# tanushreebanerjee/generative-detection

Hardware: AMD Instinct MI355X
Metric: VAE train images/s (fwd+bwd+opt) at 256x256 z=16x16x16 (higher is better)
Workload: dtype f32; 1 GPU; autoencoder_kl_16x16x16.yaml, 256x256 synthetic crops, B=32/GPU, rec+KL only (discriminator off, optimizer 0), fp32, VAE phase; global_batch=32, parallelism=dp1

## Files before the change

generative-detection_amd/csrc/bf16_common.h:

```cpp
#pragma once
#include "common.h"

typedef unsigned short bf16_t;
typedef __bf16 bf16x8 __attribute__((ext_vector_type(8)));
typedef short s16x4 __attribute__((ext_vector_type(4)));
typedef unsigned int u32x2 __attribute__((ext_vector_type(2)));

__device__ __forceinline__ float bf16_to_f32(bf16_t v) { return __uint_as_float((unsigned)v << 16); }
__device__ __forceinline__ bf16_t f32_to_bf16(float f) {
  unsigned u = __float_as_uint(f);
  if ((u & 0x7FFFFFFFu) > 0x7F800000u) return (bf16_t)((u >> 16) | 0x40);
  u += 0x7FFFu + ((u >> 16) & 1u);
  return (bf16_t)(u >> 16);
}
__device__ __forceinline__ unsigned pack_bf16x2(float lo, float hi) {
#if defined(__HIP_DEVICE_COMPILE__)
  unsigned r;
  asm("v_cvt_pk_bf16_f32 %0, %1, %2" : "=v"(r) : "v"(lo), "v"(hi));
  return r;
#else
  (void)lo; (void)hi; return 0;
#endif
}
__device__ __forceinline__ float bf16_lo(unsigned w) { return __uint_as_float(w << 16); }
__device__ __forceinline__ float bf16_hi(unsigned w) { return __uint_as_float(w & 0xFFFF0000u); }

__device__ __forceinline__ f32x16 mfma_bf16(bf16x8 a, bf16x8 b, f32x16 c) {
#if defined(__HIP_DEVICE_COMPILE__)
  return __builtin_amdgcn_mfma_f32_32x32x16_bf16(a, b, c, 0, 0, 0);
#else
  (void)a; (void)b; return c;
#endif
}
__device__ __forceinline__ bf16x8 frag_from_u32x4(u32x4 v) { return __builtin_bit_cast(bf16x8, v); }

__device__ __forceinline__ s16x4 lds_read_tr16(const bf16_t* lds_addr) {
#if defined(__HIP_DEVICE_COMPILE__)
  return __builtin_amdgcn_ds_read_tr16_b64_v4i16((s16x4 __attribute__((address_space(3)))*)lds_addr);
#else
  (void)lds_addr; return s16x4{0, 0, 0, 0};
#endif
}
__device__ __forceinline__ bf16x8 frag_from_tr(s16x4 lo, s16x4 hi) {
  typedef short s16x8 __attribute__((ext_vector_type(8)));
  s16x8 v = {lo[0], lo[1], lo[2], lo[3], hi[0], hi[1], hi[2], hi[3]};
  return __builtin_bit_cast(bf16x8, v);
}

typedef __attribute__((address_space(3))) char lds_char_t;
__device__ __forceinline__ unsigned lds_addr_of(const void* generic) { return (unsigned)(uintptr_t)(lds_char_t*)generic; }
__device__ __forceinline__ u32x4 lds_ld128(unsigned a) { return *(const __attribute__((address_space(3))) u32x4*)(uintptr_t)a; }
__device__ __forceinline__ f32x4 lds_ld128f(unsigned a) { return *(const __attribute__((address_space(3))) f32x4*)(uintptr_t)a; }
__device__ __forceinline__ void lds_st128(unsigned a, u32x4 v) { *(__attribute__((address_space(3))) u32x4*)(uintptr_t)a = v; }
__device__ __forceinline__ void lds_st128f(unsigned a, f32x4 v) { *(__attribute__((address_space(3))) f32x4*)(uintptr_t)a = v; }
__device__ __forceinline__ s16x4 lds_ld_tr(unsigned a) {
#if defined(__HIP_DEVICE_COMPILE__)
  return __builtin_amdgcn_ds_read_tr16_b64_v4i16((s16x4 __attribute__((address_space(3)))*)(uintptr_t)a);
#else
  (void)a; return s16x4{0, 0, 0, 0};
#endif
}

typedef int i32x4_t __attribute__((ext_vector_type(4)));
__device__ __forceinline__ i32x4_t rsrc_words(const void* base, unsigned bytes) {
  const uint64_t a = (uint64_t)base;
  i32x4_t r;
  r.x = (int)(unsigned)a; r.y = (int)((unsigned)(a >> 32) & 0xFFFFu); r.z = (int)bytes; r.w = 0x00020000;
  return r;
}
__device__ __forceinline__ void lds_dma16(i32x4_t rsrc, unsigned lds_dst, unsigned voff) {
#if defined(__HIP_DEVICE_COMPILE__)
  unsigned keep;
  asm volatile("s_mov_b32 %0, m0\n\ts_mov_b32 m0, %2\n\ts_nop 0\n\tbuffer_load_dwordx4 %1, %3, 0 offen lds\n\ts_mov_b32 m0, %0"
               : "=&s"(keep) : "v"(voff), "s"(lds_dst), "s"(rsrc) : "memory");
#else
  (void)rsrc; (void)lds_dst; (void)voff;
#endif
}
__device__ __forceinline__ void lds_dma16_s(i32x4_t rsrc, unsigned lds_dst, unsigned voff, unsigned soff) {
// ... 18 lines not shown
```

generative-detection_amd/csrc/conv3x3_wgrad_wino_f32.hip:

```cpp
#include "common.h"

namespace {

constexpr int CT = 16;
constexpr int RS = 128;
constexpr int OPF = 4 * CT * RS;
constexpr unsigned OOB = 0xFFFFFFF0u;

struct WgwParams {
  const float* x; const float* dy; float* slabs; float* bias_part;
  int N, H, W, Cin, Cout, TY, TX;
  int total_tiles, total_chunks, chunks_per_split, nsplit;
};

__device__ __forceinline__ float4 f4(u32x4 v) {
  return make_float4(__uint_as_float(v.x), __uint_as_float(v.y), __uint_as_float(v.z), __uint_as_float(v.w));
}
template <int A, int B>
__device__ __forceinline__ float4 f4lin(float4 x, float4 y) {
  static_assert(A >= -1 && A <= 1 && B >= -1 && B <= 1 && (A != 0 || B != 0), "coefficients are -1, 0 or 1");
  if constexpr (B == 0) return A > 0 ? x : make_float4(-x.x, -x.y, -x.z, -x.w);
  else if constexpr (A == 0) return B > 0 ? y : make_float4(-y.x, -y.y, -y.z, -y.w);
  else if constexpr (A > 0 && B > 0) return make_float4(x.x + y.x, x.y + y.y, x.z + y.z, x.w + y.w);
  else if constexpr (A > 0) return make_float4(x.x - y.x, x.y - y.y, x.z - y.z, x.w - y.w);
  else if constexpr (B > 0) return make_float4(y.x - x.x, y.y - x.y, y.z - x.z, y.w - x.w);
  else return make_float4(-x.x - y.x, -x.y - y.y, -x.z - y.z, -x.w - y.w);
}
__device__ __forceinline__ float4 f4add(float4 a, float4 b) { return make_float4(a.x + b.x, a.y + b.y, a.z + b.z, a.w + b.w); }
__device__ __forceinline__ float4 f4sub(float4 a, float4 b) { return make_float4(a.x - b.x, a.y - b.y, a.z - b.z, a.w - b.w); }

template <bool WIDE, int R>
__device__ __forceinline__ void wgw_body(const WgwParams& p, float* dsm, const int split) {
  const int tid = threadIdx.x, lane = tid & 63;
  const int wave = __builtin_amdgcn_readfirstlane(tid >> 6);
  const int cig = wave & 3, coh = wave >> 2;
  const int li = lane & 31, h = lane >> 5;
  constexpr int r = R;
  const int cib = blockIdx.y, cob = blockIdx.z;
  constexpr int ra = r == 0 ? 0 : 1, rb = r == 3 ? 3 : 2;
  constexpr int sa = r == 2 ? -1 : 1, sb = (r == 0 || r == 3) ? -1 : 1;
  constexpr int ya = r == 3 ? 0 : 1, yb = r == 0 ? 0 : (r == 1 ? 1 : -1);

  const __amdgpu_buffer_rsrc_t xrsrc = __builtin_amdgcn_make_buffer_rsrc(
      const_cast<float*>(p.x), 0, (unsigned)((int64_t)p.N * p.H * p.W * p.Cin * 4), 0x00020000);
  const __amdgpu_buffer_rsrc_t yrsrc = __builtin_amdgcn_make_buffer_rsrc(
      const_cast<float*>(p.dy), 0, (unsigned)((int64_t)p.N * p.H * p.W * p.Cout * 4), 0x00020000);

  const int chunk0 = split * p.chunks_per_split;
  const int nch = min(p.chunks_per_split, p.total_chunks - chunk0);
  const int end_tile = min(p.total_tiles, (chunk0 + nch) * CT);

  const int st = tid >> 5, sq = tid & 31;
  int tl = chunk0 * CT + st, tn, tty, ttx;
// ... 128 lines not shown
    __builtin_amdgcn_sched_barrier(0);
    mm(1); fetch_y();
    __builtin_amdgcn_sched_barrier(0);
    ldf(va, mb, 5, 1);
    __builtin_amdgcn_sched_barrier(0);
    mm(0);
    __builtin_amdgcn_sched_barrier(0);
    ldf(va, mb, 6, 0);
    __builtin_amdgcn_sched_barrier(0);
    mm(1);
    __builtin_amdgcn_sched_barrier(0);
    ldf(va, mb, 7, 1);
    __builtin_amdgcn_sched_barrier(0);
    mm(0);
    mm(1);
    __syncthreads();
  }

#pragma unroll
  for (int c = 0; c < 4; ++c) {
    float* sl = p.slabs + ((int64_t)(split * 16 + 4 * r + c) * p.Cin + cib * 128 + cig * 32) * p.Cout + cob * 128 + coh * 64 + li;
#pragma unroll
    for (int nt = 0; nt < 2; ++nt)
#pragma unroll
      for (int q = 0; q < 16; ++q) sl[(int64_t)acc_row(q, lane) * p.Cout + nt * 32] = acc[c][nt][q];
  }
  if (r == 1 && cib == 0 && p.bias_part) {
    *reinterpret_cast<float4*>(dsm + st * 128 + 4 * sq) = bias_acc;
    __syncthreads();
    if (tid < 128) {
      float s = 0.f;
#pragma unroll
      for (int t = 0; t < CT; ++t) s += dsm[t * 128 + tid];
      p.bias_part[(int64_t)split * p.Cout + cob * 128 + tid] = s;
    }
  }
}

template <bool WIDE>
__global__ __launch_bounds__(512, 2) void conv3x3_wgrad_wino_kernel(WgwParams p) {
  extern __shared__ __attribute__((aligned(16))) float dsm[];
  const int bx = blockIdx.x;
  const bool xcd_map = (p.nsplit & 7) == 0;
  const int r = xcd_map ? (bx >> 3) & 3 : bx & 3;
  const int split = xcd_map ? (bx & 7) + 8 * (bx >> 5) : bx >> 2;
  switch (r) {
    case 0: wgw_body<WIDE, 0>(p, dsm, split); break;
    case 1: wgw_body<WIDE, 1>(p, dsm, split); break;
    case 2: wgw_body<WIDE, 2>(p, dsm, split); break;
    default: wgw_body<WIDE, 3>(p, dsm, split); break;
  }
}

__global__ __launch_bounds__(256) void conv3x3_wgrad_wino_reduce_kernel(const float* __restrict__ slabs, const float* __restrict__ bias_part,
                                                                        int nsplit, int Cin, int Cout, float* __restrict__ dw, float* __restrict__ db) {
  __shared__ float part[4][16][64];
  const int pl = threadIdx.x & 63, k = threadIdx.x >> 6;
  const int idx = blockIdx.x * 64 + pl;
  const bool live = idx < Cin * Cout;
  const int co = live ? idx % Cout : 0, ci = live ? idx / Cout : 0;
  float u[16];
#pragma unroll
  for (int xi = 0; xi < 16; ++xi) u[xi] = 0.f;
  if (live)
    for (int s = k; s < nsplit; s += 4)
#pragma unroll
      for (int xi = 0; xi < 16; ++xi) u[xi] += slabs[((int64_t)(s * 16 + xi) * Cin + ci) * Cout + co];
#pragma unroll
  for (int xi = 0; xi < 16; ++xi) part[k][xi][pl] = u[xi];
  __syncthreads();
  if (k != 0) return;
  if (live) {
#pragma unroll
    for (int xi = 0; xi < 16; ++xi) u[xi] = (part[0][xi][pl] + part[1][xi][pl]) + (part[2][xi][pl] + part[3][xi][pl]);
    float t[3][4];
#pragma unroll
    for (int j = 0; j < 4; ++j) {
      const float hs = 0.5f * (u[4 + j] + u[8 + j]), hd = 0.5f * (u[4 + j] - u[8 + j]);
      t[0][j] = u[j] + hs; t[1][j] = hd; t[2][j] = hs + u[12 + j];
    }
    float* o = dw + ((int64_t)co * Cin + ci) * 9;
#pragma unroll
    for (int a = 0; a < 3; ++a) {
      const float hs = 0.5f * (t[a][1] + t[a][2]), hd = 0.5f * (t[a][1] - t[a][2]);
      o[a * 3 + 0] = t[a][0] + hs; o[a * 3 + 1] = hd; o[a * 3 + 2] = hs + t[a][3];
    }
  }
  if (db && idx < Cout) {
    float sb = 0.f;
    for (int q = 0; q < nsplit; ++q) sb += bias_part[(int64_t)q * Cout + idx];
    db[idx] = sb;
  }
}

void plan(int N, int H, int W, int Cin, int Cout, WgwParams& p) {
  p.N = N; p.H = H; p.W = W; p.Cin = Cin; p.Cout = Cout; p.TY = H / 2; p.TX = W / 2;
  p.total_tiles = N * p.TY * p.TX;
  p.total_chunks = ceil_div(p.total_tiles, CT);
  const int base = 4 * (Cin / 128) * (Cout / 128);
  int ns = std::max(1, std::min(256 / base, p.total_chunks));
  p.chunks_per_split = ceil_div(p.total_chunks, ns);
  p.nsplit = ceil_div(p.total_chunks, p.chunks_per_split);
}

}

extern "C" {

int odvae_conv3x3_wgrad_wino_supported(int N, int H, int W, int Cin, int Cout) {
  if (N <= 0 || H <= 0 || W <= 0 || H % 2 || W % 2 || Cin <= 0 || Cout <= 0 || Cin % 128 || Cout % 128) return 0;
  const int64_t px = (int64_t)N * H * W;
  if (px * Cin * 4 >= (int64_t)OOB || px * Cout * 4 >= (int64_t)OOB || px / 4 >= (1ll << 30)) return 0;
  return 1;
}

size_t odvae_conv3x3_wgrad_wino_workspace_bytes(int N, int H, int W, int Cin, int Cout) {
  if (!odvae_conv3x3_wgrad_wino_supported(N, H, W, Cin, Cout)) return 0;
  WgwParams p; plan(N, H, W, Cin, Cout, p);
  return ((size_t)p.nsplit * 16 * Cin * Cout + (size_t)p.nsplit * Cout) * sizeof(float);
}

int odvae_conv3x3_wgrad_wino_f32(const float* x, const float* dy, int N, int H, int W, int Cin, int Cout,
                                 float* dw, float* dbias, void* workspace, size_t workspace_bytes, void* stream) {
  ODVAE_CHECK_ARG(x && dy && dw, "conv3x3_wgrad_wino: null operand");
  ODVAE_CHECK_ARG(odvae_conv3x3_wgrad_wino_supported(N, H, W, Cin, Cout),
                  "conv3x3_wgrad_wino: unsupported shape N=%d H=%d W=%d Cin=%d Cout=%d (even H, W; channels in multiples of 128; "
                  "tensors below 4 GiB)", N, H, W, Cin, Cout);
  ODVAE_CHECK_ARG(((uintptr_t)x & 15) == 0 && ((uintptr_t)dy & 15) == 0, "conv3x3_wgrad_wino: x/dy must be 16-byte aligned");
  WgwParams p; plan(N, H, W, Cin, Cout, p);
  const size_t need = odvae_conv3x3_wgrad_wino_workspace_bytes(N, H, W, Cin, Cout);
  if (!workspace || workspace_bytes < need) {
    odvae_set_error("conv3x3_wgrad_wino: workspace %zu < %zu bytes", workspace_bytes, need);
    return ODVAE_ERR_WORKSPACE;
  }
  p.x = x; p.dy = dy;
  p.slabs = static_cast<float*>(workspace);
  p.bias_part = dbias ? p.slabs + (size_t)p.nsplit * 16 * Cin * Cout : nullptr;
  const size_t smem = (size_t)4 * OPF * sizeof(float);
  auto kern = p.TX >= CT ? conv3x3_wgrad_wino_kernel<true> : conv3x3_wgrad_wino_kernel<false>;
  const hipError_t e = hipFuncSetAttribute(reinterpret_cast<const void*>(kern), hipFuncAttributeMaxDynamicSharedMemorySize, (int)smem);
  if (e != hipSuccess) {
    odvae_set_error("conv3x3_wgrad_wino: hipFuncSetAttribute failed: %s", hipGetErrorString(e));
    return ODVAE_ERR_HIP;
  }
  hipStream_t s = static_cast<hipStream_t>(stream);
  hipLaunchKernelGGL(kern, dim3(4 * p.nsplit, Cin / 128, Cout / 128), dim3(512), smem, s, p);
  ODVAE_LAUNCH_CHECK("conv3x3_wgrad_wino");
  const int pairs = Cin * Cout;
  hipLaunchKernelGGL(conv3x3_wgrad_wino_reduce_kernel, dim3(ceil_div(pairs, 64)), dim3(256), 0, s,
                     p.slabs, p.bias_part, p.nsplit, Cin, Cout, dw, dbias);
  ODVAE_LAUNCH_CHECK("conv3x3_wgrad_wino_reduce");
  return ODVAE_OK;
}

}
```

generative-detection_amd/csrc/gemm_f32_split.hip:

```cpp
#include "gemm_f32_tile.h"

namespace {

using namespace gemm_tile;

constexpr unsigned PLANE_B = BM * BK * 2;
constexpr unsigned OPER_B = 3 * PLANE_B;
constexpr unsigned OOB = 0x7FFFFFF0u;
constexpr int HI = 0, MID = 1, LO = 2;

__device__ __forceinline__ unsigned tile_byte(int row, int slot) {
  const int f = ((row >> 2) & 1) | ((((row >> 1) ^ (row >> 3)) & 1) << 1);
  return (unsigned)(row * 64 + ((slot ^ f) << 4));
}

__device__ __forceinline__ unsigned cvt_pk_bf16(float first, float second) {
  typedef float f32x2 __attribute__((ext_vector_type(2)));
  typedef __bf16 bf16x2 __attribute__((ext_vector_type(2)));
  return __builtin_bit_cast(unsigned, __builtin_convertvector(f32x2{first, second}, bf16x2));
}

__device__ __forceinline__ void split8(const float (&x)[8], u32x4 (&pl)[3]) {
#pragma unroll
  for (int j = 0; j < 4; ++j) {
    const float x0 = x[2 * j], x1 = x[2 * j + 1];
    const unsigned h = cvt_pk_bf16(x0, x1);
    const float r0 = x0 - bf16_lo(h), r1 = x1 - bf16_hi(h);
    const unsigned m = cvt_pk_bf16(r0, r1);
    const float s0 = r0 - bf16_lo(m), s1 = r1 - bf16_hi(m);
    pl[HI][j] = h; pl[MID][j] = m; pl[LO][j] = cvt_pk_bf16(s0, s1);
  }
}
__device__ __forceinline__ void store_unit(unsigned lds_oper, int row, int slot, const float (&x)[8]) {
  u32x4 pl[3];
  split8(x, pl);
  const unsigned a = lds_oper + tile_byte(row, slot);
#pragma unroll
  for (int q = 0; q < 3; ++q) lds_st128(a + q * PLANE_B, pl[q]);
}

template <bool KC>
struct SplitLoader {
  __amdgpu_buffer_rsrc_t rsrc;
  unsigned voff[2];
  unsigned ld_bytes;
  int kvalid;
  float x[2][8];

  __device__ __forceinline__ void init(const float* G, int ld, int row0, int nrows, int K) {
    const int tid = threadIdx.x;
    kvalid = K;
    ld_bytes = (unsigned)ld * 4u;
    if (KC) {
      const int rows = min(BM, nrows - row0);
      const int64_t bytes = ((int64_t)(rows - 1) * ld + K) * 4;
      rsrc = __builtin_amdgcn_make_buffer_rsrc(const_cast<float*>(G) + (int64_t)row0 * ld, 0, (int)(bytes < 0x7FFFFFF0ll ? bytes : 0x7FFFFFF0ll), 0x00020000);
#pragma unroll
      for (int i = 0; i < 2; ++i) {
        const int u = tid + 256 * i;
        voff[i] = (u >> 2) < rows ? (unsigned)(((u >> 2) * ld + 8 * (u & 3)) * 4) : OOB;
      }
    } else {
      const int64_t bytes = ((int64_t)(K - 1) * ld + (nrows - row0)) * 4;
      rsrc = __builtin_amdgcn_make_buffer_rsrc(const_cast<float*>(G) + row0, 0, (int)(bytes < 0x7FFFFFF0ll ? bytes : 0x7FFFFFF0ll), 0x00020000);
      const int row = tid & 127;
      voff[0] = row0 + row < nrows ? (unsigned)((tid >> 7) * 8 * ld + row) * 4u : OOB;
      voff[1] = 0;
    }
  }
  template <bool TAIL>
  __device__ __forceinline__ void load(int k0) {
    const int tid = threadIdx.x;
    const bool tail = TAIL && k0 + BK > kvalid;
    if (KC) {
      const unsigned soff = (unsigned)__builtin_amdgcn_readfirstlane(k0) * 4u;
#pragma unroll
      for (int i = 0; i < 2; ++i)
#pragma unroll
        for (int q = 0; q < 2; ++q) {
          unsigned vo = voff[i] + 16u * q;
          if (tail && k0 + 8 * ((tid + 256 * i) & 3) + 4 * q >= kvalid) vo = OOB;
          const u32x4 v = __builtin_amdgcn_raw_buffer_load_b128(rsrc, vo, soff, 0);
          x[i][4 * q] = __uint_as_float(v.x); x[i][4 * q + 1] = __uint_as_float(v.y);
          x[i][4 * q + 2] = __uint_as_float(v.z); x[i][4 * q + 3] = __uint_as_float(v.w);
        }
// ... 173 lines not shown
```

generative-detection_amd/lib.py:

```python
import ctypes
import os
import re

import torch

_HERE = os.path.dirname(os.path.abspath(__file__))
LIB_PATH = os.path.join(_HERE, "libodvae_hip.so")
HEADER_PATH = os.path.join(os.path.dirname(_HERE), "include", "odvae_hip.h")

_c = ctypes
_P, _I, _L, _F, _Z = _c.c_void_p, _c.c_int, _c.c_int64, _c.c_float, _c.c_size_t

ABI_VERSION = 4

PROTOTYPES = {
    "odvae_last_error": (_c.c_char_p, []),
    "odvae_abi_version": (_I, []),
    "odvae_target_arch": (_c.c_char_p, []),
    "odvae_gemm_f32_workspace_bytes": (_Z, [_I, _I, _I, _I]),
    "odvae_gemm_select_staging": (_I, [_I]),
    "odvae_gemm_f32": (_I, [_I, _I, _I, _I, _I, _F, _P, _I, _L, _P, _I, _L, _P, _I, _L, _P, _P, _I, _P, _Z, _P]),
    "odvae_gemm_softmax_bwd_f32": (_I, [_I, _I, _I, _F, _P, _I, _L, _P, _I, _L, _P, _P, _L, _P, _I, _L, _I, _P]),
    "odvae_rowdot_f32": (_I, [_P, _P, _L, _I, _P, _P]),
    "odvae_attn_row_bound_f32": (_I, [_P, _I, _I, _I, _P, _P, _P, _P]),
    "odvae_gemm_exp_bound_f32": (_I, [_I, _I, _I, _F, _P, _I, _L, _P, _I, _L, _P, _L, _P, _I, _L, _I, _P]),
    "odvae_gemm_rownorm_f32": (_I, [_I, _I, _I, _P, _I, _L, _P, _I, _L, _P, _I, _L, _P, _L, _P, _I, _P]),
    "odvae_gemm_pred_f32": (_I, [_I, _I, _I, _I, _I, _F, _P, _I, _L, _P, _I, _L, _P, _I, _L, _I, _P, _P]),
    "odvae_softmax_rows_pred_f32": (_I, [_P, _P, _L, _I, _F, _P, _P, _P]),
    "odvae_rowdot_scale_f32": (_I, [_P, _P, _P, _L, _I, _P, _P, _P]),
    "odvae_gemm_softmax_bwd_scaled_f32": (_I, [_I, _I, _I, _F, _P, _I, _L, _P, _I, _L, _P, _P, _P, _L, _P, _I, _L, _I, _P]),
    "odvae_conv3x3_pack_reduce_pad": (_I, [_I]),
    "odvae_conv3x3_pack_out_pad": (_I, [_I]),
    "odvae_conv3x3_pack_floats": (_Z, [_I, _I]),
    "odvae_conv3x3_pack_f32": (_I, [_P, _I, _I, _P, _P, _P]),
    "odvae_conv3x3_up_pack_floats": (_Z, [_I, _I]),
    "odvae_conv3x3_pack_up_f32": (_I, [_P, _I, _I, _P, _P, _P]),
    "odvae_conv3x3_wino_reduce_pad": (_I, [_I]),
    "odvae_conv3x3_wino_out_pad": (_I, [_I]),
    "odvae_conv3x3_wino_pack_floats": (_Z, [_I, _I]),
    "odvae_conv3x3_pack_wino_f32": (_I, [_P, _I, _I, _P, _P, _P]),
    "odvae_conv3x3_wino_f32": (_I, [_P, _I, _I, _I, _I, _P, _I, _P, _P, _P, _I, _P]),
    "odvae_conv3x3_wino4_reduce_pad": (_I, [_I]),
    "odvae_conv3x3_wino4_out_pad": (_I, [_I]),
    "odvae_conv3x3_wino4_pack_floats": (_Z, [_I, _I]),
    "odvae_conv3x3_wino4_supported": (_I, [_I, _I, _I, _I]),
    "odvae_conv3x3_pack_wino4_f32": (_I, [_P, _I, _I, _P, _P, _P]),
    "odvae_conv3x3_pack_wino_batch": (_I, [_P, _I, _P]),
    "odvae_conv3x3_pack_wino4_batch": (_I, [_P, _I, _P]),
    "odvae_conv3x3_wino4_f32": (_I, [_P, _I, _I, _I, _I, _P, _I, _P, _P, _P, _I, _P]),
    "odvae_conv3x3_wino4_stats_chunks": (_I, [_I, _I]),
    "odvae_conv3x3_wino4_stats_f32": (_I, [_P, _I, _I, _I, _I, _P, _I, _P, _P, _P, _P, _I, _P]),
    "odvae_conv3x3_wino4_up_f32": (_I, [_P, _I, _I, _I, _I, _P, _I, _P, _P, _P, _P, _I, _P]),
    "odvae_conv3x3_wino4_pool_f32": (_I, [_P, _I, _I, _I, _I, _P, _I, _P, _P]),
    "odvae_conv3x3_wino4_gnbwd_f32": (_I, [_P, _I, _I, _I, _I, _P, _I, _P, _P, _P, _P, _P, _P, _I, _P, _P]),
    "odvae_conv3x3_f32": (_I, [_I, _P, _I, _I, _I, _I, _P, _I, _P, _P, _P, _I, _I, _I, _P]),
    "odvae_conv3x3_wgrad_workspace_bytes": (_Z, [_I, _I, _I, _I, _I, _I]),
    "odvae_conv3x3_wgrad_f32": (_I, [_I, _P, _P, _I, _I, _I, _I, _I, _I, _I, _P, _P, _P, _Z, _P]),
    "odvae_conv3x3_wgrad_wino_supported": (_I, [_I, _I, _I, _I, _I]),
    "odvae_conv3x3_wgrad_wino_workspace_bytes": (_Z, [_I, _I, _I, _I, _I]),
    "odvae_conv3x3_wgrad_wino_f32": (_I, [_P, _P, _I, _I, _I, _I, _I, _P, _P, _P, _Z, _P]),
    "odvae_groupnorm_workspace_bytes": (_Z, [_I, _I, _I, _I]),
    "odvae_groupnorm_fwd_f32": (_I, [_P, _I, _I, _I, _I, _P, _P, _F, _I, _P, _P, _P, _P, _Z, _P]),
    "odvae_groupnorm_fwd_partials_f32": (_I, [_P, _I, _I, _I, _I, _P, _P, _F, _I, _P, _P, _P, _P, _I, _P]),
    "odvae_groupnorm_apply_f32": (_I, [_P, _I, _I, _I, _I, _P, _P, _P, _P, _I, _P, _P]),
    "odvae_groupnorm_apply_bf16": (_I, [_P, _I, _I, _I, _I, _P, _P, _P, _P, _I, _P, _P]),
    "odvae_groupnorm_bwd_f32": (_I, [_P, _P, _I, _I, _I, _I, _P, _P, _P, _P, _I, _P, _P, _P, _P, _P, _Z, _P]),
    "odvae_groupnorm_bwd_partials_f32": (_I, [_P, _P, _I, _I, _I, _I, _P, _P, _P, _P, _I, _P, _P, _P, _P, _P, _I, _P, _Z, _P]),
    "odvae_groupnorm_select_backward": (_I, [_I]),
    "odvae_groupnorm_fused_timeouts": (_I, []),
    "odvae_device_health": (_I, [_P, _P, _I, _I]),
    "odvae_attn_softmax_fallbacks": (_I, [_I]),
    "odvae_softmax_rows_f32": (_I, [_P, _P, _L, _I, _F, _P]),
    "odvae_softmax_rows_bwd_f32": (_I, [_P, _P, _P, _L, _I, _F, _P]),
    "odvae_upsample2x_bwd_f32": (_I, [_P, _P, _I, _I, _I, _I, _P]),
    "odvae_rescale_minmax_f32": (_I, [_P, _P, _I, _I, _I, _P, _P, _Z, _P]),
    "odvae_gaussian_sample_f32": (_I, [_P, _P, _P, _I, _I, _I, _P]),
    "odvae_gaussian_kl_f32": (_I, [_P, _P, _I, _I, _I, _P]),
    "odvae_gaussian_bwd_f32": (_I, [_P, _P, _P, _P, _P, _I, _I, _I, _P]),
    "odvae_l1_masked_sum_f32": (_I, [_P, _P, _P, _P, _I, _I, _I, _P, _Z, _P]),
    "odvae_l1_masked_bwd_f32": (_I, [_P, _P, _P, _P, _P, _I, _I, _I, _P]),
    "odvae_colsum_workspace_bytes": (_Z, [_L, _I]),
    "odvae_colsum_f32": (_I, [_P, _L, _I, _P, _P, _Z, _P]),
    "odvae_grad_norm_f32": (_I, [_P, _L, _F, _P, _P, _Z, _P]),
    "odvae_adam_step_f32": (_I, [_P, _P, _P, _P, _L, _F, _F, _F, _F, _I, _P, _P]),
    "odvae_nhwc_to_nchw_f32": (_I, [_P, _P, _I, _I, _I, _P]),
    "odvae_mul_mask_f32": (_I, [_P, _P, _P, _L, _I, _P]),
    "odvae_latent_combine_f32": (_I, [_P, _P, _P, _P, _L, _P]),
    "odvae_im2col4x4_f32": (_I, [_P, _P, _I, _I, _I, _I, _I, _I, _I, _P]),
    "odvae_col2im4x4_f32": (_I, [_P, _P, _I, _I, _I, _I, _I, _I, _I, _P]),
    "odvae_weight4x4_reorder_f32": (_I, [_P, _P, _I, _I, _I, _P]),
    "odvae_batchnorm_workspace_bytes": (_Z, [_L, _I]),
    "odvae_batchnorm_lrelu_fwd_f32": (_I, [_P, _L, _I, _P, _P, _F, _F, _F, _I, _P, _P, _P, _P, _P, _P, _Z, _P]),
    "odvae_batchnorm_lrelu_bwd_f32": (_I, [_P, _P, _L, _I, _P, _P, _P, _P, _F, _I, _P, _P, _P, _P, _Z, _P]),
    "odvae_leaky_relu_f32": (_I, [_P, _P, _F, _L, _P]),
    "odvae_leaky_relu_bwd_f32": (_I, [_P, _P, _P, _F, _L, _P]),
    "odvae_scaling_layer_f32": (_I, [_P, _P, _P, _P, _L, _I, _I, _P]),
    "odvae_maxpool2x2_f32": (_I, [_P, _P, _I, _I, _I, _I, _P]),
    "odvae_maxpool2x2_bwd_f32": (_I, [_P, _P, _P, _P, _I, _I, _I, _I, _P]),
    "odvae_lpips_distance_f32": (_I, [_P, _P, _P, _P, _I, _I, _I, _P, _Z, _P]),
    "odvae_lpips_distance_bwd_f32": (_I, [_P, _P, _P, _P, _P, _I, _I, _I, _P]),
    "odvae_pose_losses_f32": (_I, [_P, _P, _P, _P, _P, _P, _P, _P, _I, _I, _I, _I, _I, _I, _F, _F, _P, _P, _P, _P]),
    "odvae_pose_losses_bwd_f32": (_I, [_P, _P, _P, _I, _I, _P, _P, _P]),
    "odvae_linear_workspace_bytes": (_Z, [_I, _I, _I]),
    "odvae_linear_fwd_f32": (_I, [_P, _P, _P, _I, _I, _I, _I, _P, _P, _P, _Z, _P]),
    "odvae_linear_bwd_f32": (_I, [_P, _P, _P, _P, _I, _I, _I, _I, _P, _P, _P, _P, _Z, _P]),
    "odvae_conv_bf16_reduce_pad": (_I, [_I]),
    "odvae_conv_bf16_out_pad": (_I, [_I]),
    "odvae_conv_bf16_pack_elems": (_Z, [_I, _I, _I]),
    "odvae_conv_pack_bf16": (_I, [_P, _I, _I, _I, _P, _P, _P]),
    "odvae_conv_bf16": (_I, [_I, _P, _I, _I, _I, _I, _P, _I, _P, _P, _P, _I, _I, _I, _P]),
    "odvae_conv_bf16_stats_chunks": (_I, [_I, _I]),
    "odvae_conv_bf16_stats_supported": (_I, [_I, _I]),
    "odvae_conv_bf16_stats": (_I, [_P, _I, _I, _I, _I, _P, _I, _P, _P, _P, _P, _I, _P]),
# ... 141 lines not shown
```

include/odvae_hip.h:

```cpp
#ifndef ODVAE_HIP_H
#define ODVAE_HIP_H

#include <stddef.h>
#include <stdint.h>

#ifdef __cplusplus
extern "C" {
#endif

#define ODVAE_ABI_VERSION 4
#define ODVAE_OK 0
#define ODVAE_ERR_ARG 1
#define ODVAE_ERR_WORKSPACE 2
#define ODVAE_ERR_HIP 3

const char* odvae_last_error(void);
int odvae_abi_version(void);
const char* odvae_target_arch(void);

size_t odvae_gemm_f32_workspace_bytes(int M, int N, int K, int batch);
int odvae_gemm_select_staging(int mode);
int odvae_gemm_f32(int transA, int transB, int M, int N, int K, float alpha,
                   const float* A, int lda, int64_t strideA,
                   const float* B, int ldb, int64_t strideB,
                   float* C, int ldc, int64_t strideC,
                   const float* bias, const float* residual, int batch,
                   void* workspace, size_t workspace_bytes, void* stream);

int odvae_conv3x3_pack_reduce_pad(int c_reduce);
int odvae_conv3x3_pack_out_pad(int c_out);
size_t odvae_conv3x3_pack_floats(int c_reduce, int c_out);
int odvae_conv3x3_pack_f32(const float* w_oihw, int Cout, int Cin, float* fwd_pack, float* dgrad_pack, void* stream);
size_t odvae_conv3x3_up_pack_floats(int c_reduce, int c_out);
int odvae_conv3x3_pack_up_f32(const float* w_oihw, int Cout, int Cin, float* fwd16, float* dgrad16, void* stream);
int odvae_conv3x3_f32(int mode, const float* x, int N, int Hi, int Wi, int Cin,
                      const float* wpk, int Cout, const float* bias, const float* residual,
                      float* y, int Ho, int Wo, int act , void* stream);

int odvae_conv3x3_wino_reduce_pad(int c_reduce);
int odvae_conv3x3_wino_out_pad(int c_out);
size_t odvae_conv3x3_wino_pack_floats(int c_reduce, int c_out);
int odvae_conv3x3_pack_wino_f32(const float* w_oihw, int Cout, int Cin, float* fwd_pack, float* dgrad_pack, void* stream);
int odvae_conv3x3_wino_f32(const float* x, int N, int H, int W, int Cin, const float* upk, int Cout,
                           const float* bias, const float* residual, float* y, int act , void* stream);

int odvae_conv3x3_wino4_reduce_pad(int c_reduce);
int odvae_conv3x3_wino4_out_pad(int c_out);
size_t odvae_conv3x3_wino4_pack_floats(int c_reduce, int c_out);
int odvae_conv3x3_wino4_supported(int H, int W, int Cin, int Cout);
int odvae_conv3x3_pack_wino4_f32(const float* w_oihw, int Cout, int Cin, float* fwd_pack, float* dgrad_pack, void* stream);
int odvae_conv3x3_pack_wino_batch(const void* items, int n, void* stream);
int odvae_conv3x3_pack_wino4_batch(const void* items, int n, void* stream);

int odvae_conv3x3_wino4_f32(const float* x, int N, int H, int W, int Cin, const float* upk, int Cout,
                            const float* bias, const float* residual, float* y, int act , void* stream);
int odvae_conv3x3_wino4_stats_chunks(int H, int W);
int odvae_conv3x3_wino4_stats_f32(const float* x, int N, int H, int W, int Cin, const float* upk, int Cout,
                                  const float* bias, const float* residual, float* y, float* gn_partial, int gn_groups, void* stream);
int odvae_conv3x3_wino4_up_f32(const float* x, int N, int H, int W, int Cin, const float* upk, int Cout, const float* bias,
                               const float* residual, float* y, float* gn_partial, int gn_groups, void* stream);
int odvae_conv3x3_wino4_pool_f32(const float* x, int N, int H, int W, int Cin, const float* upk, int Cout, float* y, void* stream);
int odvae_conv3x3_wino4_gnbwd_f32(const float* x, int N, int H, int W, int Cin, const float* upk, int Cout, float* y,
                                  const float* gn_x, const float* gn_mean, const float* gn_rstd, const float* gn_gamma, const float* gn_beta,
                                  int gn_groups, float* gn_partial, void* stream);

size_t odvae_conv3x3_wgrad_workspace_bytes(int mode, int N, int Ho, int Wo, int Cin, int Cout);
int odvae_conv3x3_wgrad_f32(int mode, const float* x, const float* dy, int N, int Hi, int Wi, int Cin,
                            int Ho, int Wo, int Cout, float* dw, float* dbias,
                            void* workspace, size_t workspace_bytes, void* stream);

int odvae_conv3x3_wgrad_wino_supported(int N, int H, int W, int Cin, int Cout);
size_t odvae_conv3x3_wgrad_wino_workspace_bytes(int N, int H, int W, int Cin, int Cout);
int odvae_conv3x3_wgrad_wino_f32(const float* x, const float* dy, int N, int H, int W, int Cin, int Cout,
                                 float* dw, float* dbias, void* workspace, size_t workspace_bytes, void* stream);

size_t odvae_groupnorm_workspace_bytes(int N, int HW, int C, int G);
int odvae_groupnorm_fwd_f32(const float* x, int N, int HW, int C, int G, const float* gamma, const float* beta,
                            float eps, int swish, float* y, float* mean, float* rstd,
                            void* workspace, size_t workspace_bytes, void* stream);
int odvae_groupnorm_fwd_partials_f32(const float* x, int N, int HW, int C, int G, const float* gamma, const float* beta,
                                     float eps, int swish, float* y, float* mean, float* rstd,
                                     const float* partial, int chunks, void* stream);
int odvae_groupnorm_apply_f32(const float* x, int N, int HW, int C, int G, const float* gamma, const float* beta,
                              const float* mean, const float* rstd, int swish, float* y, void* stream);
int odvae_groupnorm_apply_bf16(const void* x, int N, int HW, int C, int G, const float* gamma, const float* beta,
                               const float* mean, const float* rstd, int swish, void* y, void* stream);
int odvae_groupnorm_bwd_f32(const float* x, const float* dy, int N, int HW, int C, int G,
                            const float* gamma, const float* beta, const float* mean, const float* rstd, int swish,
                            float* dx, float* dgamma, float* dbeta, const float* dx_add,
                            void* workspace, size_t workspace_bytes, void* stream);
int odvae_groupnorm_bwd_partials_f32(const float* x, const float* dy, int N, int HW, int C, int G,
                                     const float* gamma, const float* beta, const float* mean, const float* rstd, int swish,
                                     float* dx, float* dgamma, float* dbeta, const float* dx_add, const float* partial, int chunks,
                                     void* workspace, size_t workspace_bytes, void* stream);
int odvae_groupnorm_select_backward(int mode);
int odvae_groupnorm_fused_timeouts(void);
int odvae_device_health(int* gn_timeouts, int* attn_fallbacks, int inject_gn_timeouts, int inject_attn_fallbacks);
int odvae_attn_softmax_fallbacks(int add);

int odvae_softmax_rows_f32(const float* x, float* y, int64_t rows, int cols, float scale, void* stream);
int odvae_softmax_rows_bwd_f32(const float* p, const float* dp, float* ds, int64_t rows, int cols, float scale, void* stream);
int odvae_rowdot_f32(const float* a, const float* b, int64_t rows, int cols, float* out, void* stream);
int odvae_gemm_softmax_bwd_f32(int M, int N, int K, float alpha, const float* A, int lda, int64_t strideA,
                               const float* B, int ldb, int64_t strideB, const float* P, const float* rowdot,
                               int64_t strideRow, float* dS, int ldc, int64_t strideC, int batch, void* stream);
int odvae_attn_row_bound_f32(const float* qkv, int N, int T, int C, float* bound, float* nk_scratch, int* flag, void* stream);
int odvae_gemm_exp_bound_f32(int M, int N, int K, float alpha, const float* A, int lda, int64_t strideA, const float* B, int ldb, int64_t strideB,
                             const float* rowbound, int64_t strideRow, float* E, int ldc, int64_t strideC, int batch, void* stream);
int odvae_gemm_rownorm_f32(int M, int N, int K, const float* A, int lda, int64_t strideA, const float* B, int ldb, int64_t strideB,
                           float* C, int ldc, int64_t strideC, float* rinv, int64_t strideRow, int* flag, int batch, void* stream);
int odvae_gemm_pred_f32(int transA, int transB, int M, int N, int K, float alpha, const float* A, int lda, int64_t strideA,
                        const float* B, int ldb, int64_t strideB, float* C, int ldc, int64_t strideC, int batch, const int* pred, void* stream);
int odvae_softmax_rows_pred_f32(const float* x, float* y, int64_t rows, int cols, float scale, const int* pred, float* ones, void* stream);
int odvae_rowdot_scale_f32(const float* a, const float* b, const float* row_scale, int64_t rows, int cols, float* out, float* a_scaled, void* stream);
int odvae_gemm_softmax_bwd_scaled_f32(int M, int N, int K, float alpha, const float* A, int lda, int64_t strideA,
                                      const float* B, int ldb, int64_t strideB, const float* E, const float* rowdot, const float* rinv,
                                      int64_t strideRow, float* dS, int ldc, int64_t strideC, int batch, void* stream);
int odvae_upsample2x_bwd_f32(const float* du, float* dx, int N, int H, int W, int C, void* stream);
int odvae_rescale_minmax_f32(const float* x_nchw, float* y_nhwc, int N, int C, int HW, float* minmax_out,
                             void* workspace, size_t workspace_bytes, void* stream);
int odvae_gaussian_sample_f32(const float* moments, const float* eps, float* z, int N, int HW, int Cz, void* stream);
int odvae_gaussian_kl_f32(const float* moments, float* kl, int N, int HW, int Cz, void* stream);
int odvae_gaussian_bwd_f32(const float* moments, const float* eps, const float* dz, const float* dkl,
                           float* dmoments, int N, int HW, int Cz, void* stream);
int odvae_l1_masked_sum_f32(const float* x, const float* xr, const float* mask, float* out, int N, int HW, int C,
                            void* workspace, size_t workspace_bytes, void* stream);
int odvae_l1_masked_bwd_f32(const float* x, const float* xr, const float* mask, const float* g, float* dxr,
// ... 95 lines not shown
```

Baseline: 155.3 images/s.

## Add bf16x3-split MFMA variant of Winograd conv3x3 weight-gradient kernel

Adds a new Winograd weight-gradient kernel that splits each f32 transformed operand into three bf16 planes (hi/mid/lo) and accumulates products on bf16 MFMA instructions, approximating f32 accuracy with six products per pair. Input and output-gradient tiles are fetched with buffer loads, transformed in registers and written to swizzled LDS while the MFMAs for the previous tile run, giving a software-pipelined schedule. The variant is selected by default when shapes fit (width tile divisible and tensors under the buffer size limit). A runtime selector exposes a switch back to the old path. The bf16 split trades a small accuracy loss for matrix-core throughput in place of the previous f32 path.

```diff
diff --git a/generative-detection_amd/csrc/bf16_common.h b/generative-detection_amd/csrc/bf16_common.h
--- a/generative-detection_amd/csrc/bf16_common.h
+++ b/generative-detection_amd/csrc/bf16_common.h
@@ -25,6 +25,23 @@
 __device__ __forceinline__ float bf16_lo(unsigned w) { return __uint_as_float(w << 16); }
 __device__ __forceinline__ float bf16_hi(unsigned w) { return __uint_as_float(w & 0xFFFF0000u); }
 
+__device__ __forceinline__ unsigned cvt_pk_bf16(float first, float second) {
+  typedef float f32x2 __attribute__((ext_vector_type(2)));
+  typedef __bf16 bf16x2 __attribute__((ext_vector_type(2)));
+  return __builtin_bit_cast(unsigned, __builtin_convertvector(f32x2{first, second}, bf16x2));
+}
+
+__device__ __forceinline__ void split8(const float (&x)[8], u32x4 (&pl)[3]) {
+#pragma unroll
+  for (int j = 0; j < 4; ++j) {
+    const float x0 = x[2 * j], x1 = x[2 * j + 1];
+    const unsigned h = cvt_pk_bf16(x0, x1);
+    const float r0 = x0 - bf16_lo(h), r1 = x1 - bf16_hi(h);
+    const unsigned m = cvt_pk_bf16(r0, r1);
+    const float s0 = r0 - bf16_lo(m), s1 = r1 - bf16_hi(m);
+    pl[0][j] = h; pl[1][j] = m; pl[2][j] = cvt_pk_bf16(s0, s1);
+  }
+}
 __device__ __forceinline__ f32x16 mfma_bf16(bf16x8 a, bf16x8 b, f32x16 c) {
 #if defined(__HIP_DEVICE_COMPILE__)
   return __builtin_amdgcn_mfma_f32_32x32x16_bf16(a, b, c, 0, 0, 0);
diff --git a/generative-detection_amd/csrc/conv3x3_wgrad_wino_f32.hip b/generative-detection_amd/csrc/conv3x3_wgrad_wino_f32.hip
--- a/generative-detection_amd/csrc/conv3x3_wgrad_wino_f32.hip
+++ b/generative-detection_amd/csrc/conv3x3_wgrad_wino_f32.hip
@@ -1,4 +1,5 @@
-#include "common.h"
+#include "bf16_common.h"
+#include <type_traits>
 
 namespace {
 
@@ -233,6 +234,215 @@
   }
 }
 
+constexpr unsigned SP_ROWS_B = 128 * 32;
+constexpr unsigned SP_PLANE_B = 4 * SP_ROWS_B;
+constexpr unsigned SP_OPER_B = 3 * SP_PLANE_B;
+constexpr unsigned SP_OOB = 0x7FFFFFF0u;
+constexpr int64_t SP_MAX_BYTES = 0x7F000000ll;
+
+__device__ __forceinline__ unsigned sp_byte(int row, int half) {
+  return (unsigned)(row * 32 + ((half ^ ((row >> 2) ^ (row >> 3)) & 1) << 4));
+}
+template <int A, int B>
+__device__ __forceinline__ float flin(float x, float y) {
+  static_assert(A >= -1 && A <= 1 && B >= -1 && B <= 1 && A != 0 && B != 0, "coefficients are -1 or 1");
+  if constexpr (A > 0 && B > 0) return x + y;
+  else if constexpr (A > 0) return x - y;
+  else if constexpr (B > 0) return y - x;
+  else return -x - y;
+}
+
+template <int R>
+__device__ __forceinline__ void wgs_body(const WgwParams& p, char* smem, const int split) {
+  const int tid = threadIdx.x, lane = tid & 63;
+  const int wave = __builtin_amdgcn_readfirstlane(tid >> 6);
+  const int cig = wave & 3, coh = wave >> 2;
+  const int li = lane & 31, h = lane >> 5;
+  constexpr int r = R;
+  const int cib = blockIdx.y, cob = blockIdx.z;
+  constexpr int ra = r == 0 ? 0 : 1, rb = r == 3 ? 3 : 2;
+  constexpr int sa = r == 2 ? -1 : 1, sb = (r == 0 || r == 3) ? -1 : 1;
+  constexpr int ya = r == 3 ? -1 : (r == 2 ? 1 : 0), yb = r == 0 ? -1 : (r == 2 ? 0 : 1);
+
+  const int chunk0 = split * p.chunks_per_split;
+  const int nch = min(p.chunks_per_split, p.total_chunks - chunk0);
+
+  const bool is_y = wave >= 4;
+  const int half = (tid >> 7) & 1, ch = tid & 127;
+  const int C = is_y ? p.Cout : p.Cin;
+  const __amdgpu_buffer_rsrc_t rsrc = __builtin_amdgcn_make_buffer_rsrc(
+      const_cast<float*>(is_y ? p.dy : p.x), 0, (unsigned)((int64_t)p.N * p.H * p.W * C * 4), 0x00020000);
+  const unsigned c4 = (unsigned)C * 4u;
+  const unsigned chb = (unsigned)((is_y ? cob : cib) * 128 + ch) * 4u;
+  const int row0 = is_y ? ya : ra - 1, row1 = is_y ? yb : rb - 1;
+  int g, tty, ttx, kf = 0;
+  {
+    const int t0 = chunk0 * CT;
+    g = t0 / p.TX; ttx = t0 - g * p.TX; tty = g % p.TY;
+  }
+  float ld[2][18], u[18];
+  unsigned fo[2][3];
+  auto fetch_setup = [&]() {
+    const bool live = kf < nch;
+    ++kf;
+    const int tx = ttx + 8 * half;
+    const bool cok0 = !is_y && tx > 0, cok17 = !is_y && tx + 8 < p.TX;
+    const bool rok[2] = {live && (is_y ? ya >= 0 : (ra != 0 || tty > 0)), live && (is_y ? yb >= 0 : (rb != 3 || tty < p.TY - 1))};
+    const unsigned b0 = (unsigned)((2 * g + row0) * p.W + 2 * tx) * c4 + chb;
+    const unsigned bb[2] = {b0, b0 + (unsigned)((row1 - row0) * p.W) * c4};
+#pragma unroll
+    for (int i = 0; i < 2; ++i) {
+      fo[i][0] = (rok[i] && cok0) ? bb[i] - c4 : SP_OOB;
+      fo[i][1] = rok[i] ? bb[i] : SP_OOB;
+      fo[i][2] = (rok[i] && cok17) ? bb[i] : SP_OOB;
+    }
+    ttx += CT;
+    if (ttx == p.TX) { ttx = 0; ++g; tty = tty + 1 == p.TY ? 0 : tty + 1; }
+  };
+  auto fetch_piece = [&](int n) {
+#pragma unroll
+    for (int q = 3 * n; q < 3 * n + 3; ++q) {
+      const int i = q / 18, j = q % 18;
+      const unsigned vo = j == 0 ? fo[i][0] : (j == 17 ? fo[i][2] : fo[i][1]);
+      ld[i][j] = __uint_as_float(__builtin_amdgcn_raw_buffer_load_b32(rsrc, vo, j == 0 ? 0u : (unsigned)(j - 1) * c4, 0));
+    }
+  };
+  auto transform = [&]() {
+#pragma unroll
+    for (int j = 0; j < 18; ++j) u[j] = flin<sa, sb>(ld[0][j], ld[1][j]);
+  };
+  const unsigned lds0 = lds_addr_of(smem);
+  const unsigned wr = lds0 + (is_y ? SP_OPER_B : 0u) + sp_byte(ch, half);
+  float bias_acc[8];
+#pragma unroll
+  for (int t = 0; t < 8; ++t) bias_acc[t] = 0.f;
+
+  f32x16 acc[4][2];
+#pragma unroll
+  for (int c = 0; c < 4; ++c)
+#pragma unroll
+    for (int nt = 0; nt < 2; ++nt)
+#pragma unroll
+      for (int q = 0; q < 16; ++q) acc[c][nt][q] = 0.f;
+
+  const unsigned adrA = lds0 + sp_byte(cig * 32 + li, h);
+  const unsigned adrB = lds0 + SP_OPER_B + sp_byte(coh * 64 + li, h);
+
+  auto half_phase = [&](auto pcc, auto scc, auto fetchc) {
+    constexpr int PC = decltype(pcc)::value, SC = decltype(scc)::value;
+    constexpr bool FETCH = decltype(fetchc)::value;
+    constexpr int HI = 0, MID = 1, LO = 2;
+    constexpr int ORDER[6][2] = {{LO, HI}, {HI, LO}, {MID, MID}, {MID, HI}, {HI, MID}, {HI, HI}};
+    bf16x8 a[3], b[2][3];
+    if constexpr (PC >= 0) {
+#pragma unroll
+      for (int q = 2; q >= 0; --q) {
+        a[q] = frag_from_u32x4(lds_ld128(adrA + PC * SP_ROWS_B + q * SP_PLANE_B));
+        b[0][HI + LO - q] = frag_from_u32x4(lds_ld128(adrB + PC * SP_ROWS_B + (HI + LO - q) * SP_PLANE_B));
+        b[1][HI + LO - q] = frag_from_u32x4(lds_ld128(adrB + PC * SP_ROWS_B + (HI + LO - q) * SP_PLANE_B + 1024u));
+      }
+    }
+    if constexpr (FETCH) { transform(); fetch_setup(); }
+    float x0[4], x1[4], r0[4], r1[4];
+    u32x4 pl[3];
+#pragma unroll
+    for (int i = 0; i < 12; ++i) {
+      const int j = i / 3, t = 2 * j;
+      if (i % 3 == 0) {
+        float v[2];
+#pragma unroll
+        for (int e = 0; e < 2; ++e) {
+          const float u0 = u[2 * (t + e)], u1 = u[2 * (t + e) + 1], u2 = u[2 * (t + e) + 2], u3 = u[2 * (t + e) + 3];
+          if constexpr (SC == 0) v[e] = is_y ? u1 : u0 - u2;
+          else if constexpr (SC == 1) v[e] = u1 + u2;
+          else if constexpr (SC == 2) { const float d = u2 - u1; v[e] = is_y ? -d : d; }
+          else v[e] = is_y ? -u2 : u1 - u3;
+          if constexpr (SC == 1 && r == 1) bias_acc[t + e] += v[e];
+        }
+        x0[j] = v[0]; x1[j] = v[1];
+        pl[HI][j] = cvt_pk_bf16(x0[j], x1[j]);
+        r0[j] = x0[j] - bf16_lo(pl[HI][j]);
+        asm volatile("" : "+v"(r0[j]), "+v"(pl[HI][j]));
+      } else if (i % 3 == 1) {
+        r1[j] = x1[j] - bf16_hi(pl[HI][j]);
+        pl[MID][j] = cvt_pk_bf16(r0[j], r1[j]);
+        r0[j] = r0[j] - bf16_lo(pl[MID][j]);
+        asm volatile("" : "+v"(r0[j]), "+v"(pl[MID][j]));
+      } else {
+        r1[j] = r1[j] - bf16_hi(pl[MID][j]);
+        pl[LO][j] = cvt_pk_bf16(r0[j], r1[j]);
+        asm volatile("" : "+v"(pl[LO][j]));
+      }
+      if constexpr (FETCH) fetch_piece(i);
+      if constexpr (PC >= 0) {
+        const int o = i >> 1, nt = i & 1;
+        acc[PC][nt] = mfma_bf16(a[ORDER[o][0]], b[nt][ORDER[o][1]], acc[PC][nt]);
+        __builtin_amdgcn_sched_barrier(0);
+      }
+    }
+#pragma unroll
+    for (int q = 0; q < 3; ++q) lds_st128(wr + SC * SP_ROWS_B + q * SP_PLANE_B, pl[q]);
+    if constexpr (PC >= 0) __builtin_amdgcn_sched_barrier(0);
+  };
+  using IN = std::integral_constant<int, -1>;
+  using I0 = std::integral_constant<int, 0>; using I1 = std::integral_constant<int, 1>;
+  using I2 = std::integral_constant<int, 2>; using I3 = std::integral_constant<int, 3>;
+
+  fetch_setup();
+#pragma unroll
+  for (int n = 0; n < 12; ++n) fetch_piece(n);
+  half_phase(IN{}, I0{}, std::true_type{});
+  half_phase(IN{}, I1{}, std::false_type{});
+  __syncthreads();
+  for (int k = 0; k < nch; ++k) {
+    half_phase(I0{}, I2{}, std::false_type{});
+    half_phase(I1{}, I3{}, std::false_type{});
+    __syncthreads();
+    half_phase(I2{}, I0{}, std::true_type{});
+    half_phase(I3{}, I1{}, std::false_type{});
+    __syncthreads();
+  }
+
+#pragma unroll
+  for (int c = 0; c < 4; ++c) {
+    float* sl = p.slabs + ((int64_t)(split * 16 + 4 * r + c) * p.Cin + cib * 128 + cig * 32) * p.Cout + cob * 128 + coh * 64 + li;
+#pragma unroll
+    for (int nt = 0; nt < 2; ++nt)
+#pragma unroll
+      for (int q = 0; q < 16; ++q) sl[(int64_t)acc_row(q, lane) * p.Cout + nt * 32] = acc[c][nt][q];
+  }
+  if constexpr (r == 1) {
+    if (cib == 0 && p.bias_part) {
+      float* bs = reinterpret_cast<float*>(smem);
+      if (is_y) {
+#pragma unroll
+        for (int t = 0; t < 8; ++t) bs[(8 * half + t) * 128 + ch] = bias_acc[t];
+      }
+      __syncthreads();
+      if (tid < 128) {
+        float s = 0.f;
+#pragma unroll
+        for (int t = 0; t < CT; ++t) s += bs[t * 128 + tid];
+        p.bias_part[(int64_t)split * p.Cout + cob * 128 + tid] = s;
+      }
+    }
+  }
+}
+
+__global__ __launch_bounds__(512, 2) void conv3x3_wgrad_wino_split_kernel(WgwParams p) {
+  extern __shared__ __attribute__((aligned(16))) char ssm[];
+  const int bx = blockIdx.x;
+  const bool xcd_map = (p.nsplit & 7) == 0;
+  const int r = xcd_map ? (bx >> 3) & 3 : bx & 3;
+  const int split = xcd_map ? (bx & 7) + 8 * (bx >> 5) : bx >> 2;
+  switch (r) {
+    case 0: wgs_body<0>(p, ssm, split); break;
+    case 1: wgs_body<1>(p, ssm, split); break;
+    case 2: wgs_body<2>(p, ssm, split); break;
+    default: wgs_body<3>(p, ssm, split); break;
+  }
+}
+
 __global__ __launch_bounds__(256) void conv3x3_wgrad_wino_reduce_kernel(const float* __restrict__ slabs, const float* __restrict__ bias_part,
                                                                         int nsplit, int Cin, int Cout, float* __restrict__ dw, float* __restrict__ db) {
   __shared__ float part[4][16][64];
@@ -284,9 +494,22 @@
   p.nsplit = ceil_div(p.total_chunks, p.chunks_per_split);
 }
 
+bool split_supported(int N, int H, int W, int Cin, int Cout) {
+  const int64_t px = (int64_t)N * H * W;
+  return (W / 2) % CT == 0 && px * Cin * 4 < SP_MAX_BYTES && px * Cout * 4 < SP_MAX_BYTES;
+}
+bool split_by_shape(int N, int H, int W, int Cin, int Cout) { return split_supported(N, H, W, Cin, Cout); }
+int g_form = -1;
+
 }
 
 extern "C" {
+
+int odvae_conv3x3_wgrad_wino_select(int form) {
+  const int prev = g_form;
+  g_form = form < 0 ? -1 : (form > 1 ? 1 : form);
+  return prev;
+}
 
 int odvae_conv3x3_wgrad_wino_supported(int N, int H, int W, int Cin, int Cout) {
   if (N <= 0 || H <= 0 || W <= 0 || H % 2 || W % 2 || Cin <= 0 || Cout <= 0 || Cin % 128 || Cout % 128) return 0;
@@ -317,8 +540,9 @@
   p.x = x; p.dy = dy;
   p.slabs = static_cast<float*>(workspace);
   p.bias_part = dbias ? p.slabs + (size_t)p.nsplit * 16 * Cin * Cout : nullptr;
-  const size_t smem = (size_t)4 * OPF * sizeof(float);
-  auto kern = p.TX >= CT ? conv3x3_wgrad_wino_kernel<true> : conv3x3_wgrad_wino_kernel<false>;
+  const bool split = g_form != 0 && split_supported(N, H, W, Cin, Cout) && (g_form == 1 || split_by_shape(N, H, W, Cin, Cout));
+  const size_t smem = split ? (size_t)2 * SP_OPER_B : (size_t)4 * OPF * sizeof(float);
+  auto kern = split ? conv3x3_wgrad_wino_split_kernel : (p.TX >= CT ? conv3x3_wgrad_wino_kernel<true> : conv3x3_wgrad_wino_kernel<false>);
   const hipError_t e = hipFuncSetAttribute(reinterpret_cast<const void*>(kern), hipFuncAttributeMaxDynamicSharedMemorySize, (int)smem);
   if (e != hipSuccess) {
     odvae_set_error("conv3x3_wgrad_wino: hipFuncSetAttribute failed: %s", hipGetErrorString(e));
diff --git a/generative-detection_amd/csrc/gemm_f32_split.hip b/generative-detection_amd/csrc/gemm_f32_split.hip
--- a/generative-detection_amd/csrc/gemm_f32_split.hip
+++ b/generative-detection_amd/csrc/gemm_f32_split.hip
@@ -14,23 +14,6 @@
   return (unsigned)(row * 64 + ((slot ^ f) << 4));
 }
 
-__device__ __forceinline__ unsigned cvt_pk_bf16(float first, float second) {
-  typedef float f32x2 __attribute__((ext_vector_type(2)));
-  typedef __bf16 bf16x2 __attribute__((ext_vector_type(2)));
-  return __builtin_bit_cast(unsigned, __builtin_convertvector(f32x2{first, second}, bf16x2));
-}
-
-__device__ __forceinline__ void split8(const float (&x)[8], u32x4 (&pl)[3]) {
-#pragma unroll
-  for (int j = 0; j < 4; ++j) {
-    const float x0 = x[2 * j], x1 = x[2 * j + 1];
-    const unsigned h = cvt_pk_bf16(x0, x1);
-    const float r0 = x0 - bf16_lo(h), r1 = x1 - bf16_hi(h);
-    const unsigned m = cvt_pk_bf16(r0, r1);
-    const float s0 = r0 - bf16_lo(m), s1 = r1 - bf16_hi(m);
-    pl[HI][j] = h; pl[MID][j] = m; pl[LO][j] = cvt_pk_bf16(s0, s1);
-  }
-}
 __device__ __forceinline__ void store_unit(unsigned lds_oper, int row, int slot, const float (&x)[8]) {
   u32x4 pl[3];
   split8(x, pl);
diff --git a/generative-detection_amd/lib.py b/generative-detection_amd/lib.py
--- a/generative-detection_amd/lib.py
+++ b/generative-detection_amd/lib.py
@@ -59,6 +59,7 @@
     "odvae_conv3x3_wgrad_wino_supported": (_I, [_I, _I, _I, _I, _I]),
     "odvae_conv3x3_wgrad_wino_workspace_bytes": (_Z, [_I, _I, _I, _I, _I]),
     "odvae_conv3x3_wgrad_wino_f32": (_I, [_P, _P, _I, _I, _I, _I, _I, _P, _P, _P, _Z, _P]),
+    "odvae_conv3x3_wgrad_wino_select": (_I, [_I]),
     "odvae_groupnorm_workspace_bytes": (_Z, [_I, _I, _I, _I]),
     "odvae_groupnorm_fwd_f32": (_I, [_P, _I, _I, _I, _I, _P, _P, _F, _I, _P, _P, _P, _P, _Z, _P]),
     "odvae_groupnorm_fwd_partials_f32": (_I, [_P, _I, _I, _I, _I, _P, _P, _F, _I, _P, _P, _P, _P, _I, _P]),
diff --git a/include/odvae_hip.h b/include/odvae_hip.h
--- a/include/odvae_hip.h
+++ b/include/odvae_hip.h
@@ -73,6 +73,7 @@
 size_t odvae_conv3x3_wgrad_wino_workspace_bytes(int N, int H, int W, int Cin, int Cout);
 int odvae_conv3x3_wgrad_wino_f32(const float* x, const float* dy, int N, int H, int W, int Cin, int Cout,
                                  float* dw, float* dbias, void* workspace, size_t workspace_bytes, void* stream);
+int odvae_conv3x3_wgrad_wino_select(int form);
 
 size_t odvae_groupnorm_workspace_bytes(int N, int HW, int C, int G);
 int odvae_groupnorm_fwd_f32(const float* x, int N, int HW, int C, int G, const float* gamma, const float* beta,
```

New measurement: 160.8 images/s (median of 6 runs). +3.6%, better.
